# 666DZY666/micronet

Hardware: NVIDIA H100
Metric: qat_step_images_per_sec (higher is better)
Workload: dtype f32 (bf16 tensor-core products of exact integer levels / exact bf16 pieces, fp32 accumulate)

## Files before the change

### include/micronet_b200.h

```cpp
#ifndef MICRONET_B200_H
#define MICRONET_B200_H

#include <stdint.h>

#ifdef __cplusplus
extern "C" {
#endif

typedef void* mnb_stream_t;

#define MNB_E_ARG (-1)
#define MNB_E_UNSUPPORTED (-2)

int mnb_version(void);
const char* mnb_last_error(void);
int64_t mnb_launch_count(void);

typedef struct {
  int32_t batch, in_c, in_h, in_w;
  int32_t out_c, ker_h, ker_w;
  int32_t stride_h, stride_w, pad_h, pad_w, dil_h, dil_w, groups;
} mnb_conv_shape;

#define MNB_ACT_DOREFA 1
// ... 218 lines not shown
                           const mnb_act_qparams* qp, int32_t relu, float* out, const mnb_pk_post* post, mnb_stream_t stream);
int mnb_pk_conv_post_plan(const mnb_conv_shape* s, int32_t terms_a, int32_t terms_w, int32_t cpu, const mnb_pk_post* post,
                          int32_t* out, int32_t n);
int64_t mnb_pk_i8_act_bytes(int32_t batch, int32_t channels, int32_t h, int32_t w);
int mnb_pk_i8_pack_act(const float* x, int32_t batch, int32_t channels, int32_t h, int32_t w, const mnb_act_qparams* qp,
                       int32_t phase_split, int32_t relu, void* out_pk, mnb_stream_t stream);
int mnb_pk_i8_conv_plan(const mnb_conv_shape* s, int32_t* out, int32_t n);
int64_t mnb_pk_i8_wimage_bytes(const mnb_conv_shape* s);
int mnb_pk_i8_pack_weight(const mnb_conv_shape* s, const int16_t* w_int, void* w_img, mnb_stream_t stream);
int mnb_pk_i8_conv(const mnb_conv_shape* s, const void* a_pk, const void* w_img, const float* n_scale, const float* a_scale,
                   float a_scale_const, const float* bias, float* out, const mnb_pk_post* post, int32_t* err_flag,
                   mnb_stream_t stream);
int mnb_quant_add_pack_i8_fwd(const float* a, const float* b, int32_t batch, int32_t channels, int32_t h, int32_t w,
                              const mnb_act_qparams* qp, int32_t relu, float* out, const mnb_pk_post* post, mnb_stream_t stream);
int mnb_bn_relu_quant_pack_i8_fwd(const float* x, int32_t batch, int32_t channels, int32_t hw, const float* mean,
                                  const float* invstd, const float* gamma, const float* beta, const mnb_act_qparams* qp,
                                  int32_t out_shuffle_groups, void* x_packed, mnb_stream_t stream);
int mnb_pk_plane_maxpool(const void* in_pk, int32_t batch, int32_t channels, int32_t h, int32_t w, int32_t k, int32_t s, int32_t p,
                         int32_t int8, void* out_pk, mnb_stream_t stream);
int mnb_pk_plane_maxpool_requant(const void* in_pk, int32_t batch, int32_t channels, int32_t h, int32_t w, int32_t k, int32_t s,
                                 int32_t p, int32_t int8, const mnb_act_qparams* q_in, const mnb_act_qparams* q_out, void* out_pk,
                                 mnb_stream_t stream);
int mnb_pk_plane_maxpool_terms(const void* in_pk, int32_t batch, int32_t channels, int32_t h, int32_t w, int32_t k, int32_t s,
                               int32_t p, int32_t terms, void* out_pk, mnb_stream_t stream);
int mnb_bn_relu_pack_terms_fwd(const float* x, int32_t batch, int32_t channels, int32_t hw, const float* mean,
                               const float* invstd, const float* gamma, const float* beta, int32_t relu,
                               int32_t out_shuffle_groups, int32_t terms, void* x_packed, mnb_stream_t stream);
int64_t mnb_pk_wgrad_scratch_bytes(const mnb_conv_shape* s, int32_t terms_dy, int32_t terms_x);
int mnb_pk_wgrad(const mnb_conv_shape* s, const void* dy_pk, int32_t terms_dy, const void* x_pk, int32_t terms_x,
                 const float* a_scale, const float* kdiv, float* dw, void* scratch, int32_t* err_flag, mnb_stream_t stream);
int mnb_pk_wgrad_taps_plan(const mnb_conv_shape* s, int32_t terms_dy, int32_t terms_x, int32_t* out, int32_t n);
int mnb_pk_wgrad_taps(const mnb_conv_shape* s, const void* dy_pk, int32_t terms_dy, const void* x_pk, int32_t terms_x,
                      const float* a_scale, const float* kdiv, float* dw, void* scratch, int32_t* err_flag, mnb_stream_t stream);
int mnb_pk_gc3_plan(const mnb_conv_shape* s, int32_t mode, int32_t terms_a, int32_t terms_w, int32_t* out, int32_t n);
int mnb_pk_gc3_conv(const mnb_conv_shape* s, int32_t mode, const void* a_pk, int32_t terms_a, const void* w_img, int32_t terms_w,
                    const float* n_scale, const float* a_scale, float a_scale_const, const float* bias, const uint8_t* bits8,
                    float gain, float* out, int32_t* err_flag, mnb_stream_t stream);
int mnb_pk_gc3_conv_codes(const mnb_conv_shape* s, const void* a_pk, int32_t terms_a, const void* w_img, int32_t terms_w,
                          const float* n_scale, const float* a_scale, float a_scale_const, const float* bias, int32_t level_bound,
                          int16_t* codes, float* dec, int32_t* err_flag, mnb_stream_t stream);

int mnb_xnor_supported(const mnb_conv_shape* s);
int64_t mnb_xnor_act_bytes(int32_t batch, int32_t channels, int32_t h, int32_t w, int32_t groups);
int mnb_xnor_pack_act(const float* x, int32_t batch, int32_t channels, int32_t h, int32_t w, int32_t groups, void* out_bits,
                      mnb_stream_t stream);
int64_t mnb_xnor_wimage_bytes(const mnb_conv_shape* s);
int mnb_xnor_pack_weight(const mnb_conv_shape* s, const int16_t* w_int, void* w_img, mnb_stream_t stream);
int mnb_xnor_conv_fwd(const mnb_conv_shape* s, const void* a_bits, const void* w_img, const float* alpha, const float* bias,
                      float* y, mnb_stream_t stream);
#define MNB_XNOR_BITS 0
#define MNB_XNOR_PM1_BF16 1
typedef struct mnb_xnor_post {
  int32_t format;
  int32_t out_groups;
  int32_t shuffle_groups;
  int32_t pool2;
  const float* bn_mean;
  const float* bn_invstd;
  const float* bn_gamma;
  const float* bn_beta;
} mnb_xnor_post;
int64_t mnb_xnor_post_bytes(const mnb_conv_shape* s, const mnb_xnor_post* post);
int mnb_xnor_conv_post(const mnb_conv_shape* s, const void* a_bits, const void* w_img, const float* alpha, const float* bias,
                       const mnb_xnor_post* post, void* out, mnb_stream_t stream);
int mnb_xnor_pack_act_post(const float* x, int32_t batch, int32_t channels, int32_t h, int32_t w, const mnb_xnor_post* post,
                           void* out_bits, mnb_stream_t stream);
// ... 38 lines not shown
```

### micronet_b200/_lib.py

```python
from __future__ import annotations

import ctypes as C
import os

import torch

_HERE = os.path.dirname(os.path.abspath(__file__))
LIB_PATH = os.path.join(_HERE, "lib", "libmicronet_b200.so")

ACT_DOREFA, ACT_IAO, ACT_SIGN = 1, 2, 3


class ConvShape(C.Structure):
    _fields_ = [(n, C.c_int32) for n in (
        "batch", "in_c", "in_h", "in_w", "out_c", "ker_h", "ker_w", "stride_h", "stride_w",
        "pad_h", "pad_w", "dil_h", "dil_w", "groups")]


class ActQParams(C.Structure):
    _fields_ = [("mode", C.c_int32), ("bits", C.c_int32), ("qmin", C.c_int32), ("qmax", C.c_int32),
                ("q_type", C.c_int32), ("scale", C.c_void_p), ("zero_point", C.c_void_p),
                ("obs_min", C.c_void_p), ("obs_max", C.c_void_p)]


# ... 83 lines not shown
    "mnb_pk_pack_weight": (C.c_int, [_SHAPE, _I, _I, _I, _P, _P, _P, _P, _P]),
    "mnb_pk_conv": (C.c_int, [_SHAPE, _I, _P, _I, _P, _I, _P, _P, C.c_float, _P, _P, C.c_float, _P, _P, _P]),
    "mnb_bn_sign_bwd_pack": (C.c_int, [_P, _P, _P, _I, _I, _I, _P, _P, _P, _P, _P, _I, _P, _I, _P, _P, _P]),
    "mnb_bn_sign_pool_bwd_pack": (C.c_int, [_P, _P, _P, _P, _I, _I, _I, _I, _P, _P, _P, _P, _P, _I, _P, _I, _P, _P]),
    "mnb_pk_conv_post": (C.c_int, [_SHAPE, _P, _I, _P, _I, _P, _P, C.c_float, _P, _P, C.POINTER(PkPost), _P, _P]),
    "mnb_pk_conv_post_plan": (C.c_int, [_SHAPE, _I, _I, _I, C.POINTER(PkPost), _P, _I]),
    "mnb_pk_conv_codes": (C.c_int, [_SHAPE, _P, _I, _P, _I, _P, _P, C.c_float, _P, _I, _P, _P, _P, _P]),
    "mnb_codes_decode": (C.c_int, [_P, _P, _I, _I, _I, _P, _P]),
    "mnb_bn_batch_stats_codes": (C.c_int, [_P, _P, _I, _I, _I, _D, _D, _P, _P, _P, _P, _P, _P]),
    "mnb_bn_sign_fwd_packed_codes": (C.c_int, [_P, _P, _I, _I, _I, _P, _P, _P, _P, _I, _P, _P, _P, _P]),
    "mnb_bn_sign_bwd_codes": (C.c_int, [_P, _P, _P, _P, _I, _I, _I, _P, _P, _P, _I, _I, _P, _P, _P, _P, _P, _P]),
    "mnb_bn_sign_pool_fwd_codes": (C.c_int, [_P, _P, _I, _I, _I, _I, _P, _P, _P, _P, _I, _P, _P, _P, _P]),
    "mnb_bn_sign_pool_bwd_codes": (C.c_int, [_P, _P, _P, _P, _P, _I, _I, _I, _I, _P, _P, _P, _I, _I, _P, _P, _P, _P, _P, _P]),
    "mnb_bn_sign_bwd_pack_codes": (C.c_int, [_P, _P, _P, _P, _I, _I, _I, _P, _P, _P, _P, _P, _I, _P, _I, _P, _P, _P]),
    "mnb_bn_sign_pool_bwd_pack_codes": (C.c_int, [_P, _P, _P, _P, _P, _I, _I, _I, _I, _P, _P, _P, _P, _P, _I, _P, _I, _P,
                                                  _P]),
    "mnb_quant_add_pack_fwd": (C.c_int, [_P, _P, _I, _I, _I, _I, _ACTQ, _I, _P, C.POINTER(PkPost), _P]),
    "mnb_pk_i8_act_bytes": (_L, [_I, _I, _I, _I]),
    "mnb_pk_i8_pack_act": (C.c_int, [_P, _I, _I, _I, _I, _ACTQ, _I, _I, _P, _P]),
    "mnb_pk_i8_conv_plan": (C.c_int, [_SHAPE, _P, _I]),
    "mnb_pk_i8_wimage_bytes": (_L, [_SHAPE]),
    "mnb_pk_i8_pack_weight": (C.c_int, [_SHAPE, _P, _P, _P]),
    "mnb_pk_i8_conv": (C.c_int, [_SHAPE, _P, _P, _P, _P, C.c_float, _P, _P, C.POINTER(PkPost), _P, _P]),
    "mnb_quant_add_pack_i8_fwd": (C.c_int, [_P, _P, _I, _I, _I, _I, _ACTQ, _I, _P, C.POINTER(PkPost), _P]),
    "mnb_bn_relu_quant_pack_i8_fwd": (C.c_int, [_P, _I, _I, _I, _P, _P, _P, _P, _ACTQ, _I, _P, _P]),
    "mnb_pk_plane_maxpool": (C.c_int, [_P, _I, _I, _I, _I, _I, _I, _I, _I, _P, _P]),
    "mnb_pk_plane_maxpool_requant": (C.c_int, [_P, _I, _I, _I, _I, _I, _I, _I, _I, _ACTQ, _ACTQ, _P, _P]),
    "mnb_pk_plane_maxpool_terms": (C.c_int, [_P, _I, _I, _I, _I, _I, _I, _I, _I, _P, _P]),
    "mnb_bn_relu_pack_terms_fwd": (C.c_int, [_P, _I, _I, _I, _P, _P, _P, _P, _I, _I, _I, _P, _P]),
    "mnb_pk_wgrad_scratch_bytes": (_L, [_SHAPE, _I, _I]),
    "mnb_pk_wgrad": (C.c_int, [_SHAPE, _P, _I, _P, _I, _P, _P, _P, _P, _P, _P]),
    "mnb_pk_wgrad_taps_plan": (C.c_int, [_SHAPE, _I, _I, _P, _I]),
    "mnb_pk_wgrad_taps": (C.c_int, [_SHAPE, _P, _I, _P, _I, _P, _P, _P, _P, _P, _P]),
    "mnb_pk_gc3_plan": (C.c_int, [_SHAPE, _I, _I, _I, _P, _I]),
    "mnb_pk_gc3_conv": (C.c_int, [_SHAPE, _I, _P, _I, _P, _I, _P, _P, C.c_float, _P, _P, C.c_float, _P, _P, _P]),
    "mnb_pk_gc3_conv_codes": (C.c_int, [_SHAPE, _P, _I, _P, _I, _P, _P, C.c_float, _P, _I, _P, _P, _P, _P]),
    "mnb_xnor_supported": (C.c_int, [_SHAPE]),
    "mnb_xnor_act_bytes": (_L, [_I, _I, _I, _I, _I]),
    "mnb_xnor_pack_act": (C.c_int, [_P, _I, _I, _I, _I, _I, _P, _P]),
    "mnb_xnor_wimage_bytes": (_L, [_SHAPE]),
    "mnb_xnor_pack_weight": (C.c_int, [_SHAPE, _P, _P, _P]),
    "mnb_xnor_conv_fwd": (C.c_int, [_SHAPE, _P, _P, _P, _P, _P, _P]),
    "mnb_xnor_post_bytes": (_L, [_SHAPE, C.POINTER(XnorPost)]),
    "mnb_xnor_conv_post": (C.c_int, [_SHAPE, _P, _P, _P, _P, C.POINTER(XnorPost), _P, _P]),
    "mnb_xnor_pack_act_post": (C.c_int, [_P, _I, _I, _I, _I, C.POINTER(XnorPost), _P, _P]),
    "mnb_xnor_plan": (C.c_int, [_SHAPE, C.POINTER(XnorPost), _P]),
    "mnb_b1_supported": (C.c_int, [_SHAPE]),
    "mnb_b1_act_bytes": (_L, [_I, _I, _I, _I, _I]),
    "mnb_b1_pack_act": (C.c_int, [_P, _I, _I, _I, _I, _I, _P, _P]),
    "mnb_b1_pack_act_post": (C.c_int, [_P, _I, _I, _I, _I, C.POINTER(XnorPost), _P, _P]),
    "mnb_b1_wimage_bytes": (_L, [_SHAPE]),
    "mnb_b1_pack_weight": (C.c_int, [_SHAPE, _P, _P, _P]),
    "mnb_b1_conv_fwd": (C.c_int, [_SHAPE, _P, _P, _P, _P, _P, _P, _P]),
    "mnb_b1_plan": (C.c_int, [_SHAPE, C.POINTER(XnorPost), _P]),
    "mnb_b1_post_bytes": (_L, [_SHAPE, C.POINTER(XnorPost)]),
    "mnb_b1_conv_post": (C.c_int, [_SHAPE, _P, _P, _P, _P, C.POINTER(XnorPost), _P, _P, _P]),
    "mnb_b1_plane_maxpool": (C.c_int, [_P, _I, _I, _I, _I, _I, _I, _I, _I, _P, _P]),
    "mnb_set_tc_profile_buffer": (None, [_P]),
    "mnb_selftest_mma_rate": (C.c_int, [_I, _I, _I, _I, _I, _P, _P, _P]),
    "mnb_selftest_umma": (C.c_int, [_P, _P, _P, _I, _I, _I, _P, _P]),
    "mnb_selftest_tma3d": (C.c_int, [_P, C.POINTER(C.c_int64), C.POINTER(C.c_int32), C.POINTER(C.c_int32), _P, _P, _P]),
}

_lib = None


# ... 42 lines not shown
            raise TypeError(f"micronet_b200: fp32 tensors only (the reference's QAT modules are fp32), got {t.dtype}")


def launch_count() -> int:
    return int(load().mnb_launch_count())


_errflags = {}


def tc_err_flag(device):
    key = (device.type, device.index)
    if key not in _errflags:
        _errflags[key] = torch.zeros(1, dtype=torch.int32, device=device)
    return _errflags[key]


def tc_check(device=None):
    for key, flag in _errflags.items():
        code = int(flag.item())
        if code:
            raise RuntimeError(f"micronet_b200: tensor-core pipeline wait timed out (code {code}) on {key}")


E_UNSUPPORTED = -2
KEEP_DEBUG = False
USE_TC = os.environ.get("MNB_DISABLE_TC", "0") != "1"
PK_MODE = os.environ.get("MNB_PK", "auto")
PK_TERMS = int(os.environ.get("MNB_PK_TERMS", "3"))
PK_TERMS_BWD = int(os.environ.get("MNB_PK_TERMS_BWD", "2"))
PK_WBWTAB = os.environ.get("MNB_PK_WBWTAB", "1") == "1"
PK_WG_TAPS = os.environ.get("MNB_PK_WG_TAPS", "1") != "0"
PK_GC3 = os.environ.get("MNB_PK_GC3", "1") != "0"

XNOR_MODE = os.environ.get("MNB_XNOR", "auto")

PLANE_ONLY = os.environ.get("MNB_PLANE_ONLY", "1") == "1"

_scratch = {}


def scratch(device, rows=1):
    lib = load()
    need = int(lib.mnb_observe_scratch_bytes(0, int(rows)))
    key = (device.type, device.index)
    buf = _scratch.get(key)
    if buf is None or buf.numel() < need:
        buf = torch.zeros(max(need, 1 << 20), dtype=torch.uint8, device=device)
        _scratch[key] = buf
    return buf
```

### micronet_b200/csrc/mnb_pk.cu

```cuda
#include <cuda.h>
#include <cuda_bf16.h>

#include <algorithm>
#include <cstdlib>
#include <cstring>

#include "mnb_common.cuh"
#include "mnb_tc.cuh"

namespace pk {

constexpr int MAXST = 8;
constexpr int MAXTAP = 64, MAXTMPL = 16, MAXY = 4, MAXPAIR = 6, MAXPROG = 512;
constexpr int kSmemBudget = 227 * 1024 - 3072;
constexpr int kNtSizes[] = {16, 32, 48, 64, 96, 128};

struct Tmpl { int kph, tap0, ntap, blk_off, blk_bytes; };

struct Plan {
  int mode;
  int B, G, R, S, stride;
  int HA, WA, C8A, nkph;
  int kg, ng, NOUT;
  int OHr, OWr, OH, OW, omul, ny;
// ... 1703 lines not shown
      const uint32_t nsubs = min(p.NI, p.nsub - stg * p.NI);
      tc::wg_fence();
#pragma unroll
      for (int t = 0; t < kTapsN; ++t) tc::fence_acc(acc[t]);
      for (uint32_t si = 0; si < nsubs; ++si) {
        const uint32_t s16 = slot * p.stage16 + si * p.sub16;
        for (uint32_t j = 0; j < p.ksteps; ++j) {
          for (uint32_t pr = 0; pr < p.npairs; ++pr) {
            const uint64_t ad = a_hi | (uint64_t)(a_lo0 + s16 + 16u * j + p.pair_a16[pr]);
            const uint32_t bb = b_lo0 + s16 + 16u * j + p.pair_b16[pr];
#pragma unroll
            for (int t = 0; t < kTapsN; ++t) tc::Mma<32>::bf16<1, 1>(acc[t], ad, b_hi | (uint64_t)(bb + p.tap16[t]), 1);
          }
        }
      }
      tc::wg_commit();
      tc::wg_wait<0>();
#pragma unroll
      for (int t = 0; t < kTapsN; ++t) tc::fence_acc(acc[t]);
      __syncwarp();
      if (lane == 0) tc::mbar_arrive(&sh.empty[slot]);
      if (++slot == p.nstage) { slot = 0; ph ^= 1u; }
    }
    float* dst = p.partial + ((int64_t)split * gridDim.x + blk) * (int64_t)(kTapsN * 64 * 128);
    const int kr = 64 * wg + 16 * w4 + (lane >> 2), cb = 32 * wg + 2 * (lane & 3);
#pragma unroll
    for (int t = 0; t < kTapsN; ++t)
#pragma unroll
      for (int j = 0; j < 4; ++j) {
        if ((j >> 1) != (w4 >> 1)) continue;
#pragma unroll
        for (int e = 0; e < 4; ++e) dst[(int64_t)(t * 64 + cb + 8 * j + (e & 1)) * 128 + kr + 8 * (e >> 1)] = acc[t][4 * j + e];
      }
  }
  __syncthreads();
}

constexpr int kGc3MaxMb = 8;
constexpr int kGc3MaxProg = 128;
constexpr int kGc3Cons = 3;
constexpr int kGc3Threads = 128 * (1 + kGc3Cons);
constexpr int kGc3SmemBudget = 227 * 1024 - 4096;
constexpr int kGc3TmaRegs = 40, kGc3MmaRegs = 152;
__host__ __device__ constexpr int gc3_max_mb(int nt) { return nt == 32 ? 6 : kGc3MaxMb; }

struct Gc3Plan {
  Plan pl;
  int GB, nblk, TB, n_tiles, cpb, BW, THH, npos, nmb, plane, SP;
  int a_box_bytes, a_piece_bytes, stage_bytes, nstage, w_bytes, stg_bytes, off_stage, off_stg, off_rowmap, smem_bytes;
  int nprog;
  uint32_t prog[kGc3MaxProg];
  int16_t chain[kGc3MaxProg][4];
};

struct Gc3Params {
  uint32_t prog[kGc3MaxProg];
  int nprog, mode, TA, GB, ng, kg8, NOUT, B, TB, n_tiles, cpb, nmb, npos, BW, THH, OH, OW, plane, SP, C8O, wlo, hlo;
  int a_box_bytes, a_piece_bytes, stage_bytes, nstage, w_bytes, img_bytes, stg_bytes, off_stage, off_stg, off_rowmap, smem_bytes;
  const uint8_t* w_img;
  const float* n_scale;
  const float* a_scale;
  float a_scale_const;
  const float* bias;
  const uint8_t* bits8;
  float gain;
  float* out;
// ... 1022 lines not shown
  if (int e = make_wgt_plan(s, terms_dy, terms_x, pl)) return e;
  WgtParams p;
  memset(&p, 0, sizeof(p));
  p.stg_per_split = pl.stg_per_split; p.nstg_total = pl.nstg_total; p.NI = pl.NI; p.nsub = pl.nsub; p.ksteps = pl.rows_dy / 16;
  p.npairs = pl.npairs; p.nstage = pl.nstage; p.stage16 = pl.stage_bytes >> 4; p.sub16 = pl.sub_bytes >> 4;
  p.dy_sbo = (uint32_t)pl.rows_dy * 16u; p.x_sbo = (uint32_t)pl.rows_x * 16u; p.x_off16 = (pl.TA * pl.dy_bytes) >> 4;
  for (int i = 0; i < pl.npairs; ++i) {
    p.pair_a16[i] = (uint32_t)(pl.pair_a[i] * pl.dy_bytes) >> 4;
    p.pair_b16[i] = (uint32_t)(pl.pair_b[i] * pl.x_bytes) >> 4;
  }
  for (int t = 0; t < kTapsN; ++t) p.tap16[t] = (uint32_t)pl.tap_off[t];
  p.row_tiles = pl.row_tiles; p.TA = pl.TA; p.TX = pl.TX; p.TH = pl.TH; p.hlo = pl.hlo; p.wlo = pl.wlo;
  p.stage_bytes = pl.stage_bytes; p.sub_bytes = pl.sub_bytes; p.dy_bytes = pl.dy_bytes; p.x_bytes = pl.x_bytes;
  p.dy_box_bytes = pl.dy_box_bytes; p.x_box_bytes = pl.x_box_bytes; p.smem_bytes = pl.smem_bytes;
  p.partial = reinterpret_cast<float*>(scratch); p.err = err_flag;
  CUtensorMap tdy[3], tx[3];
  const int64_t dy_plane = (int64_t)pl.B * pl.K8 * pl.P * pl.Q * 16;
  const int64_t x_plane = (int64_t)pl.B * pl.C8X * pl.HX * pl.WX * 16;
  for (int t = 0; t < 3; ++t) {
    if (int e = make_pk_tmap(&tdy[t], dy_pk, dy_plane, t < pl.TA ? t : 0, pl.B, pl.K8, pl.P, pl.Q, pl.BW, pl.TH, 1, 16)) return e;
    if (int e = make_pk_tmap(&tx[t], x_pk, x_plane, t < pl.TX ? t : 0, pl.B, pl.C8X, pl.HX, pl.WX, pl.BW, pl.THH, 1, 8)) return e;
  }
  if (int e = set_max_smem(pk_wgrad_taps_kernel, kSmemBudget)) return e;
  cudaStream_t st = (cudaStream_t)stream;
  pk_wgrad_taps_kernel<<<dim3(pl.G, pl.splits), kWgtThreads, pl.smem_bytes, st>>>(tdy[0], tdy[1], tdy[2], tx[0], tx[1], tx[2], p);
  const dim3 rgrid(kTapsCin * kTapsN, 1, pl.G * kTapsGm);
  wg_reduce_kernel<<<rgrid, 128, 0, st>>>(p.partial, pl.splits, pl.G, kTapsGm, 1, 1, kTapsN, pl.Nc, kTapsCout, kTapsCin, kTapsCout,
                                          kTapsCin, a_scale, kdiv, dw);
  MNB_LAUNCHED(2);
  return 0;
}


extern "C" int mnb_pk_gc3_plan(const mnb_conv_shape* s, int32_t mode, int32_t terms_a, int32_t terms_w, int32_t* out, int32_t n) {
  static pk::Gc3Plan g;
  if (int e = pk::make_gc3_plan(s, mode, terms_a, terms_w, g)) return e;
  if (out) {
    const int v[10] = {g.GB, g.TB, g.nmb, g.nstage, g.smem_bytes, g.nblk * g.cpb, g.n_tiles, g.nprog, g.pl.Nt, pk::kGc3Cons};
    for (int i = 0; i < std::min(n, 10); ++i) out[i] = v[i];
    for (int i = 10; i < n && (i - 10) / 4 < g.nprog; ++i) out[i] = g.chain[(i - 10) / 4][(i - 10) % 4];
  }
  return 0;
}

static int pk_gc3_impl(const mnb_conv_shape* s, int32_t mode, const void* a_pk, int32_t terms_a, const void* w_img, int32_t terms_w,
                       const float* n_scale, const float* a_scale, float a_scale_const, const float* bias, const uint8_t* bits8,
                       float gain, float* out, int16_t* codes, float* dec, int32_t* err_flag, mnb_stream_t stream) {
  using namespace pk;
  MNB_REQUIRE(s && a_pk && w_img && (out != nullptr) != (codes != nullptr) && err_flag, "NULL pk_gc3 pointer");
  static Gc3Plan g;
  if (int e = make_gc3_plan(s, mode, terms_a, terms_w, g)) return e;
  MNB_REQUIRE(g.nstage % kGc3Cons == 0, "pk gc3: %d stages are not a whole number per MMA warpgroup", g.nstage);
  const Plan& pl = g.pl;
  auto al16 = [](const void* q) { return (reinterpret_cast<uintptr_t>(q) & 15) == 0; };
  if (!al16(a_pk) || !al16(w_img) || !al16(out ? (const void*)out : (const void*)codes))
    return mnb_fail(MNB_E_UNSUPPORTED, "pk gc3: operands and output must be 16-byte aligned");
  static Gc3Params p;
  memset(&p, 0, sizeof(p));
  for (int i = 0; i < g.nprog; ++i) p.prog[i] = g.prog[i];
  p.nprog = g.nprog; p.mode = mode; p.TA = terms_a; p.GB = g.GB; p.ng = pl.ng; p.kg8 = pl.kg / 8; p.NOUT = pl.NOUT; p.B = pl.B;
  p.TB = g.TB; p.n_tiles = g.n_tiles; p.cpb = g.cpb; p.nmb = g.nmb; p.npos = g.npos; p.BW = g.BW; p.THH = g.THH; p.OH = pl.OHr;
  p.OW = pl.OWr; p.plane = g.plane; p.SP = g.SP; p.C8O = ceil_div(pl.NOUT, 8); p.wlo = pl.wlo; p.hlo = pl.hlo;
  p.a_box_bytes = g.a_box_bytes; p.a_piece_bytes = g.a_piece_bytes; p.stage_bytes = g.stage_bytes; p.nstage = g.nstage;
  p.w_bytes = g.w_bytes; p.img_bytes = pl.img_bytes[0]; p.stg_bytes = g.stg_bytes; p.off_stage = g.off_stage; p.off_stg = g.off_stg;
  p.off_rowmap = g.off_rowmap; p.smem_bytes = g.smem_bytes;
  p.w_img = reinterpret_cast<const uint8_t*>(w_img);
// ... 38 lines not shown
```

### micronet_b200/functional.py

```python
from __future__ import annotations

import ctypes as C

import torch
from torch.autograd import Function

from . import _lib as L


class KernelTimer:

    def __init__(self):
        self.records = []

    def run(self, kind, sh, fn):
        a, b = torch.cuda.Event(enable_timing=True), torch.cuda.Event(enable_timing=True)
        a.record()
        rc = fn()
        b.record()
        self.records.append((kind, tuple(getattr(sh, f) for f, _ in sh._fields_), a, b))
        return rc

    def summary(self):
        out = {}
# ... 293 lines not shown
            y._mnb_codes = (codes, dec)
    if rc == L.E_UNSUPPORTED:
        rc = _timed("fwd_pk", sh, lambda: PK.run_conv(sh, 0, x_pk, ta, w_img, tw, y,
                                                      n_scale=w_scale if w_int is not None else None, a_scale=a_scale,
                                                      a_scale_const=a_const, bias=bias))
    if rc == L.E_UNSUPPORTED:
        return False
    L.check(rc, "pk_conv fwd")
    ctx.pk_x, ctx.pk_ta, ctx.pk_bits8, ctx.pk_prepacked = x_pk, ta, bits8, prepacked is not None
    ctx.pk_gain = 0.1 if (spec is not None and spec.mode == L.ACT_DOREFA) else 1.0
    ctx.pk_wg_scale = None
    if spec is not None:
        ctx.pk_wg_scale = a_scale if spec.mode == L.ACT_IAO else _dorefa_scale_tensor(spec.bits, x.device)
    if spec is None and w_int is not None and need_dw and not PK.padded(sh.out_c, sh.groups):
        y._mnb_pk_conv = (w_scale if need_dx else None, Tb)
    return True


def _pk_backward(ctx, dy):
    from . import pk as PK
    sh = ctx.sh
    T = min(L.PK_TERMS, L.PK_TERMS_BWD)
    int_w = ctx.w_int is not None
    need_dx, need_dw = ctx.needs_input_grad[0], ctx.needs_input_grad[1]
    fold = int_w and need_dx
    pre = getattr(dy, "_mnb_pk_dy", None)
    if pre is not None:
        if pre[1] != T or (pre[2] is not None) != fold or PK.padded(sh.out_c, sh.groups):
            raise RuntimeError("micronet_b200: packed gradient operand does not match this layer's backward configuration")
        dy_pk = pre[0]
    else:
        dy_pk, _ = PK.pack_act(dy, None, T, ch_scale=ctx.w_scale if fold else None, groups=sh.groups)
    dx = dwq = None
    if need_dx:
        tw = 1 if int_w else T
        w_img = PK.pack_weight(sh, 1, T, tw, w_int=ctx.w_int, w_f32=None if int_w else ctx.wq,
                               kzero=ctx.w_scale if int_w else None)
        dx = torch.empty((sh.batch, sh.in_c, sh.in_h, sh.in_w), dtype=torch.float32, device=dy.device)
        plain_gain = ctx.pk_gain if ctx.pk_prepacked else 1.0
        L.check(_timed("dgrad_pk", sh, lambda: PK.run_conv(sh, 1, dy_pk, T, w_img, tw, dx, bits8=ctx.pk_bits8, gain=ctx.pk_gain,
                                                           a_scale_const=plain_gain)), "pk_conv dgrad")
    if need_dw:
        dwq = torch.empty_like(ctx.wq)
        tx = min(ctx.pk_ta, T)
        kdiv = ctx.w_scale if fold else None
        L.check(_timed("wgrad_pk", sh, lambda: PK.run_wgrad(sh, dy_pk, T, ctx.pk_x, tx, dwq, a_scale=ctx.pk_wg_scale,
                                                            kdiv=kdiv)), "pk_wgrad")
    return dx, dwq


def _xnor_forward(x, w_int, w_scale, bias, sh, y, groups):
    from . import xnor as XN
    if not (XN.supported(sh) and (L.XNOR_MODE == "all" or xnor_preferred(sh, getattr(x, "_mnb_pk_pm1", None) is not None))):
        return False
    a_bits = XN.pack_act(materialized(x), groups)
    rc = _timed("fwd_xnor", sh, lambda: XN.conv(sh, a_bits, XN.pack_weight(sh, w_int), y, alpha=w_scale, bias=bias))
    if rc == L.E_UNSUPPORTED:
        return False
    L.check(rc, "xnor_conv_fwd")
    return True


def _save_unpacked(ctx, x, spec, codes, bits, keep_x):
    if spec is not None and (ctx.needs_input_grad[0] or ctx.needs_input_grad[1]):
        spec = spec.frozen()
    ctx.spec, ctx.codes, ctx.bits = spec, codes, bits
    ctx.x = x if keep_x else None


def _act_operands(spec, codes, x):
    ops = L.ConvOperands()
    if codes is None:
        ops.a_f32 = x.data_ptr()
        return ops
    ops.a_codes, ops.a_offset = codes.data_ptr(), spec.code_offset
    if spec.mode == L.ACT_IAO:
        ops.a_offset_zp, ops.a_scale = L.ptr(spec.zero_point), L.ptr(spec.scale)
    elif spec.mode == L.ACT_DOREFA:
# ... 559 lines not shown
```

### micronet_b200/pk.py

```python
from __future__ import annotations

import ctypes as C

import torch

from . import _lib as L

_plan_cache = {}


def _key(sh):
    return tuple(getattr(sh, f) for f, _ in sh._fields_)


def supported(sh, mode, terms_a, terms_w):
    k = ("c", _key(sh), mode, terms_a, terms_w)
    if k not in _plan_cache:
        _plan_cache[k] = L.load().mnb_pk_conv_plan(C.byref(sh), mode, terms_a, terms_w, None) == 0
    return _plan_cache[k]


def segmented(sh, mode, terms_a, terms_w):
    k = ("s", _key(sh), mode, terms_a, terms_w)
    if k not in _plan_cache:
# ... 211 lines not shown
    lib = L.load()
    nbytes = int(lib.mnb_pk_wgrad_scratch_bytes(C.byref(sh), terms_dy, terms_x))
    if nbytes < 0:
        return L.E_UNSUPPORTED
    ws = torch.empty(max(nbytes, 16), dtype=torch.uint8, device=dw.device)
    return lib.mnb_pk_wgrad(C.byref(sh), dy_pk.data_ptr(), terms_dy, x_pk.data_ptr(), terms_x, L.ptr(a_scale),
                            L.ptr(kdiv), dw.data_ptr(), ws.data_ptr(), L.tc_err_flag(dw.device).data_ptr(), L.stream())


def wgrad_taps_plan(sh, terms_dy, terms_x):
    k = ("wt", _key(sh), terms_dy, terms_x)
    if k not in _plan_cache:
        out = (C.c_int32 * 12)()
        ok = L.load().mnb_pk_wgrad_taps_plan(C.byref(sh), terms_dy, terms_x, out, 12) == 0
        names = ("blocks", "splits", "NI", "nstage", "BW", "TH", "stg_per_split", "smem_bytes", "acc_regs")
        plan = None
        if ok:
            plan = dict(zip(names, out[:9]))
            plan["scratch_bytes"] = out[9] | (out[10] << 31)
            plan["npairs"] = out[11]
        _plan_cache[k] = plan
    return _plan_cache[k]


def wgrad_taps(sh, dy_pk, terms_dy, x_pk, terms_x, dw, a_scale=None, kdiv=None):
    plan = wgrad_taps_plan(sh, terms_dy, terms_x)
    if plan is None:
        return L.E_UNSUPPORTED
    ws = torch.empty(plan["scratch_bytes"], dtype=torch.uint8, device=dw.device)
    return L.load().mnb_pk_wgrad_taps(C.byref(sh), dy_pk.data_ptr(), terms_dy, x_pk.data_ptr(), terms_x, L.ptr(a_scale),
                                      L.ptr(kdiv), dw.data_ptr(), ws.data_ptr(), L.tc_err_flag(dw.device).data_ptr(), L.stream())


def gc3_plan(sh, mode, terms_a, terms_w):
    k = ("g3", _key(sh), mode, terms_a, terms_w)
    if k not in _plan_cache:
        out = (C.c_int32 * (10 + 4 * 128))()
        ok = L.load().mnb_pk_gc3_plan(C.byref(sh), mode, terms_a, terms_w, out, len(out)) == 0
        plan = None
        if ok:
            names = ("groups_per_block", "images_per_tile", "m_blocks", "nstage", "smem_bytes", "ctas", "tiles", "chain_len",
                     "Nt", "mma_warpgroups")
            plan = dict(zip(names, out[:10]))
            plan["chain"] = [tuple(out[10 + 4 * i:14 + 4 * i]) for i in range(plan["chain_len"])]
        _plan_cache[k] = plan
    return _plan_cache[k]


def gc3_conv(sh, mode, a_pk, terms_a, w_img, terms_w, out, n_scale=None, a_scale=None, a_scale_const=1.0, bias=None,
             bits8=None, gain=1.0):
    return L.load().mnb_pk_gc3_conv(C.byref(sh), mode, a_pk.data_ptr(), terms_a, w_img.data_ptr(), terms_w, L.ptr(n_scale),
                                    L.ptr(a_scale), float(a_scale_const), L.ptr(bias), L.ptr(bits8), float(gain),
                                    out.data_ptr(), L.tc_err_flag(out.device).data_ptr(), L.stream())


def gc3_conv_codes(sh, a_pk, w_img, codes, dec, n_scale=None, a_scale=None, a_scale_const=1.0, bias=None, level_bound=1):
    return L.load().mnb_pk_gc3_conv_codes(C.byref(sh), a_pk.data_ptr(), 1, w_img.data_ptr(), 1, L.ptr(n_scale), L.ptr(a_scale),
                                          float(a_scale_const), L.ptr(bias), int(level_bound), codes.data_ptr(), dec.data_ptr(),
                                          L.tc_err_flag(codes.device).data_ptr(), L.stream())


def run_conv(sh, mode, a_pk, terms_a, w_img, terms_w, out, **epilogue):
    if L.PK_GC3 and gc3_plan(sh, mode, terms_a, terms_w) is not None:
        rc = gc3_conv(sh, mode, a_pk, terms_a, w_img, terms_w, out, **epilogue)
        if rc != L.E_UNSUPPORTED:
            return rc
    return conv(sh, mode, a_pk, terms_a, w_img, terms_w, out, **epilogue)


def run_conv_codes(sh, a_pk, w_img, codes, dec, **epilogue):
    if L.PK_GC3 and gc3_plan(sh, 0, 1, 1) is not None:
        rc = gc3_conv_codes(sh, a_pk, w_img, codes, dec, **epilogue)
        if rc != L.E_UNSUPPORTED:
            return rc
    return conv_codes(sh, a_pk, w_img, codes, dec, **epilogue)


def run_wgrad(sh, dy_pk, terms_dy, x_pk, terms_x, dw, a_scale=None, kdiv=None):
    fn = wgrad_taps if L.PK_WG_TAPS and wgrad_taps_plan(sh, terms_dy, terms_x) is not None else wgrad
    return fn(sh, dy_pk, terms_dy, x_pk, terms_x, dw, a_scale=a_scale, kdiv=kdiv)
```

Measured before the change: 41270.

## Fuse 1x1 conv data-gradient and weight-gradient into one warp-specialized kernel

```diff
diff --git a/harness/pk_bwd1x1_probe.py b/harness/pk_bwd1x1_probe.py
--- /dev/null
+++ b/harness/pk_bwd1x1_probe.py
@@ -0,0 +1,74 @@
+import argparse
+import json
+
+import torch
+
+from harness.wgrad_taps_probe import card
+from micronet_b200 import _lib as L, pk as PK
+
+SHAPES = {"L1/L2 256->256 g2 @32": (256, 256, 32, 32, 256, 2), "L4/L5 512->512 g4 @16": (256, 512, 16, 16, 512, 4),
+          "L7 1024->1024 g8 @8": (256, 1024, 8, 8, 1024, 8)}
+
+
+def main():
+    ap = argparse.ArgumentParser()
+    ap.add_argument("--iters", type=int, default=50)
+    ap.add_argument("--rounds", type=int, default=5)
+    args = ap.parse_args()
+    dev = torch.device("cuda:0")
+    out = {"card": card(), "layers": {}}
+    for name, (B, Cc, H, W, K, G) in SHAPES.items():
+        sh = L.ConvShape(B, Cc, H, W, K, 1, 1, 1, 1, 0, 0, 1, 1, G)
+        plan = PK.bwd1x1_plan(sh, 2, 1, 1)
+        g = torch.Generator().manual_seed(7)
+        ops = []
+        for _ in range(4):
+            dy = torch.randn(B, K, H, W, generator=g).to(dev)
+            x = torch.randint(0, 2, (B, Cc, H, W), generator=g).float().mul_(2).sub_(1).to(dev)
+            w_int = torch.randint(-1, 2, (K, Cc // G, 1, 1), generator=g).to(torch.int16).to(dev)
+            ops.append((PK.pack_act(dy, None, 2, groups=G)[0], PK.pack_act(x, None, 1, groups=G)[0],
+                        PK.pack_weight(sh, 1, 2, 1, w_int=w_int)))
+        res = {k: (torch.empty(B, Cc, H, W, device=dev), torch.empty(K, Cc // G, 1, 1, device=dev)) for k in ("sep", "fused")}
+
+        def sep(dy_pk, x_pk, w_img, dx, dw):
+            L.check(PK.conv(sh, 1, dy_pk, 2, w_img, 1, dx, a_scale_const=0.25), "pk_conv dgrad")
+            L.check(PK.wgrad(sh, dy_pk, 2, x_pk, 1, dw), "pk_wgrad")
+
+        def fused(dy_pk, x_pk, w_img, dx, dw):
+            L.check(PK.bwd1x1(sh, dy_pk, 2, x_pk, 1, w_img, 1, dx, dw, a_scale_const=0.25), "pk_bwd1x1")
+
+        fns = {"sep": sep, "fused": fused}
+
+        def window(k):
+            a, b = torch.cuda.Event(enable_timing=True), torch.cuda.Event(enable_timing=True)
+            a.record()
+            for i in range(args.iters):
+                fns[k](*ops[i % 4], *res[k])
+            b.record()
+            torch.cuda.synchronize()
+            return a.elapsed_time(b) * 1e3 / args.iters
+
+        for k in fns:
+            window(k)
+        t = {k: [] for k in fns}
+        for _ in range(args.rounds):
+            for k in fns:
+                t[k].append(window(k))
+        L.tc_check()
+        med = {k: sorted(v)[len(v) // 2] for k, v in t.items()}
+        n_out = B * K * H * W
+        dy_b, x_b, dx_b = n_out * 4, B * Cc * H * W * 2, B * Cc * H * W * 4
+        w_b = ops[0][2].numel()
+        part_b = plan["scratch_bytes"] * 2
+        bytes_ = {"sep": 2 * dy_b + x_b + w_b + dx_b + part_b, "fused": dy_b + x_b + w_b + dx_b + part_b}
+        same = all(torch.equal(res["sep"][i].view(torch.int32), res["fused"][i].view(torch.int32)) for i in range(2))
+        out["layers"][name] = {
+            "sep_us": med["sep"], "fused_us": med["fused"], "speedup": med["sep"] / med["fused"],
+            "sep_GBps": bytes_["sep"] / med["sep"] * 1e-3, "fused_GBps": bytes_["fused"] / med["fused"] * 1e-3,
+            "sep_bytes": bytes_["sep"], "fused_bytes": bytes_["fused"],
+            "sep_windows_us": t["sep"], "fused_windows_us": t["fused"], "byte_equal": same, "plan": plan}
+    print(json.dumps(out, indent=1))
+
+
+if __name__ == "__main__":
+    main()
diff --git a/include/micronet_b200.h b/include/micronet_b200.h
--- a/include/micronet_b200.h
+++ b/include/micronet_b200.h
@@ -274,6 +274,10 @@
 int mnb_pk_wgrad_taps_plan(const mnb_conv_shape* s, int32_t terms_dy, int32_t terms_x, int32_t* out, int32_t n);
 int mnb_pk_wgrad_taps(const mnb_conv_shape* s, const void* dy_pk, int32_t terms_dy, const void* x_pk, int32_t terms_x,
                       const float* a_scale, const float* kdiv, float* dw, void* scratch, int32_t* err_flag, mnb_stream_t stream);
+int mnb_pk_bwd1x1_plan(const mnb_conv_shape* s, int32_t terms_dy, int32_t terms_x, int32_t terms_w, int32_t* out, int32_t n);
+int mnb_pk_bwd1x1(const mnb_conv_shape* s, const void* dy_pk, int32_t terms_dy, const void* x_pk, int32_t terms_x,
+                  const void* w_img, int32_t terms_w, float a_scale_const, const uint8_t* bits8, float gain, float* dx,
+                  const float* a_scale, const float* kdiv, float* dw, void* scratch, int32_t* err_flag, mnb_stream_t stream);
 int mnb_pk_gc3_plan(const mnb_conv_shape* s, int32_t mode, int32_t terms_a, int32_t terms_w, int32_t* out, int32_t n);
 int mnb_pk_gc3_conv(const mnb_conv_shape* s, int32_t mode, const void* a_pk, int32_t terms_a, const void* w_img, int32_t terms_w,
                     const float* n_scale, const float* a_scale, float a_scale_const, const float* bias, const uint8_t* bits8,
diff --git a/micronet_b200/_lib.py b/micronet_b200/_lib.py
--- a/micronet_b200/_lib.py
+++ b/micronet_b200/_lib.py
@@ -139,6 +139,8 @@
     "mnb_pk_wgrad": (C.c_int, [_SHAPE, _P, _I, _P, _I, _P, _P, _P, _P, _P, _P]),
     "mnb_pk_wgrad_taps_plan": (C.c_int, [_SHAPE, _I, _I, _P, _I]),
     "mnb_pk_wgrad_taps": (C.c_int, [_SHAPE, _P, _I, _P, _I, _P, _P, _P, _P, _P, _P]),
+    "mnb_pk_bwd1x1_plan": (C.c_int, [_SHAPE, _I, _I, _I, _P, _I]),
+    "mnb_pk_bwd1x1": (C.c_int, [_SHAPE, _P, _I, _P, _I, _P, _I, C.c_float, _P, C.c_float, _P, _P, _P, _P, _P, _P, _P]),
     "mnb_pk_gc3_plan": (C.c_int, [_SHAPE, _I, _I, _I, _P, _I]),
     "mnb_pk_gc3_conv": (C.c_int, [_SHAPE, _I, _P, _I, _P, _I, _P, _P, C.c_float, _P, _P, C.c_float, _P, _P, _P]),
     "mnb_pk_gc3_conv_codes": (C.c_int, [_SHAPE, _P, _I, _P, _I, _P, _P, C.c_float, _P, _I, _P, _P, _P, _P]),
@@ -247,6 +249,7 @@
 PK_WBWTAB = os.environ.get("MNB_PK_WBWTAB", "1") == "1"
 PK_WG_TAPS = os.environ.get("MNB_PK_WG_TAPS", "1") != "0"
 PK_GC3 = os.environ.get("MNB_PK_GC3", "1") != "0"
+PK_BWD1X1 = os.environ.get("MNB_PK_BWD1X1", "1") != "0"
 
 XNOR_MODE = os.environ.get("MNB_XNOR", "auto")
 
diff --git a/micronet_b200/csrc/mnb_pk.cu b/micronet_b200/csrc/mnb_pk.cu
--- a/micronet_b200/csrc/mnb_pk.cu
+++ b/micronet_b200/csrc/mnb_pk.cu
@@ -1759,6 +1759,192 @@
 #pragma unroll
         for (int e = 0; e < 4; ++e) dst[(int64_t)(t * 64 + cb + 8 * j + (e & 1)) * 128 + kr + 8 * (e >> 1)] = acc[t][4 * j + e];
       }
+  }
+  __syncthreads();
+}
+
+constexpr int kBwdThreads = 384;
+constexpr int kBwdRows = 64;
+constexpr int kBwdProg = 64;
+constexpr int kBwdTmaRegs = 40, kBwdMmaRegs = 232;
+
+struct BwdPlan {
+  WgPlan wg;
+  Plan dg;
+  int nprog, off_w, w_bytes, nstage, smem_bytes;
+};
+
+static int make_bwd_plan(const mnb_conv_shape* s, int TA, int TX, int TW, BwdPlan& b) {
+  MNB_REQUIRE(s != nullptr, "conv shape is NULL");
+  MNB_REQUIRE(TA >= 1 && TA <= 3 && TX >= 1 && TX <= 3 && TW >= 1 && TW <= 3, "term counts must be 1..3");
+  memset(&b, 0, sizeof(b));
+  const int C = s->in_c, K = s->out_c, G = s->groups;
+  MNB_REQUIRE(s->batch > 0 && C > 0 && K > 0 && s->in_h > 0 && s->in_w > 0 && G > 0 && C % G == 0 && K % G == 0,
+              "bad conv shape");
+  auto no = [](const char* why) { return mnb_fail(MNB_E_UNSUPPORTED, "pk bwd1x1: %s", why); };
+  if (s->ker_h != 1 || s->ker_w != 1) return no("filter is not 1x1");
+  if (s->stride_h != 1 || s->stride_w != 1 || s->dil_h != 1 || s->dil_w != 1) return no("stride or dilation != 1");
+  if (s->pad_h != 0 || s->pad_w != 0) return no("padding != 0");
+  if (C / G > 128 || K / G > 128) return no("more than 128 channels per group");
+  if (G > 1 && ((C / G) % 8 || (K / G) % 8)) return no("group-padded operand planes");
+  if (int e = make_wg_plan(s, TA, TX, b.wg)) return e;
+  if (int e = make_plan(s, 1, TA, TW, b.dg)) return e;
+  const WgPlan& w = b.wg;
+  const Plan& d = b.dg;
+  if (w.gm != 1 || w.n_ktiles != 1 || w.n_ctiles != 1 || w.n_tg != 1) return no("weight-gradient block is not one whole group");
+  if (w.rows_dy != kBwdRows) return no("sub-block raster is not 64 positions");
+  if (d.n_ntiles != 1 || d.Nt != w.Nc || d.Nt % 32) return no("data-gradient N tile differs from the weight-gradient tile");
+  if (d.segmented) return no("segmented data-gradient plan");
+  if (d.chunks * d.ksteps * 16 > 128) return no("data-gradient K-steps beyond the dy box");
+  b.nprog = d.chunks * d.npairs * d.ksteps;
+  if (d.ny != 1 || d.ntmpl[0] != 1 || b.nprog > kBwdProg)
+    return mnb_fail(MNB_E_ARG, "pk bwd1x1: data-gradient plan with %d templates, %d MMAs", d.ntmpl[0], b.nprog);
+  b.w_bytes = round_up(d.img_bytes[0], 1024);
+  b.nstage = std::min(MAXST, (kSmemBudget - 1024 - b.w_bytes) / w.stage_bytes);
+  if (b.nstage < 2) return no("fewer than two stages fit next to the weight image");
+  b.off_w = b.nstage * w.stage_bytes + 1024;
+  b.smem_bytes = b.off_w + b.w_bytes;
+  return 0;
+}
+
+struct BwdParams {
+  uint32_t stg_per_split, nstg_total, NI, nsub, ksteps, npairs, nstage, stage16, sub16, dy_sbo, x_sbo, x_off16;
+  uint32_t pair_a16[MAXPAIR], pair_b16[MAXPAIR];
+  int row_tiles, TA, TX, TH, stage_bytes, sub_bytes, dy_bytes, x_bytes, dy_box_bytes, x_box_bytes, smem_bytes, cout_g8, cin_g8;
+  float* partial;
+  uint32_t nprog, dg_lbo, w_lbo, off_w, w_bytes, img_bytes;
+  uint32_t prog[kBwdProg];
+  const uint8_t* w_img;
+  int B, P, Q, BW, C, cin_g, C8O;
+  float a_scale_const, gain;
+  float bias0;
+  const uint8_t* bits8;
+  float* dx;
+  int* err;
+};
+
+template <int NC>
+__global__ void __launch_bounds__(kBwdThreads, 1)
+pk_bwd1x1_kernel(const __grid_constant__ CUtensorMap dy0, const __grid_constant__ CUtensorMap dy1,
+                 const __grid_constant__ CUtensorMap dy2, const __grid_constant__ CUtensorMap x0,
+                 const __grid_constant__ CUtensorMap x1, const __grid_constant__ CUtensorMap x2,
+                 const __grid_constant__ BwdParams p) {
+  extern __shared__ __align__(1024) uint8_t smem[];
+  __shared__ WgShared sh;
+  __shared__ uint64_t wbar;
+  const int tid = threadIdx.x, warp = tid >> 5, lane = tid & 31;
+  if (tid == 0) {
+    for (int i = 0; i < MAXST; ++i) { tc::mbar_init(&sh.full[i], 1); tc::mbar_init(&sh.empty[i], 8); }
+    tc::mbar_init(&wbar, 1);
+    sh.abort = 0;
+    tc::fence_barrier_init();
+    tc::prefetch_tmap(&dy0); tc::prefetch_tmap(&x0);
+  }
+  for (int i = tid; i < (int)p.off_w / 16; i += kBwdThreads) reinterpret_cast<uint4*>(smem)[i] = make_uint4(0, 0, 0, 0);
+  tc::fence_proxy_async_smem();
+  __syncthreads();
+  const int g = blockIdx.x, split = blockIdx.y;
+  const uint32_t stg0 = (uint32_t)split * p.stg_per_split, stg1 = min(p.nstg_total, stg0 + p.stg_per_split);
+
+  if (warp < 4) {
+    asm volatile("setmaxnreg.dec.sync.aligned.u32 %0;" ::"n"(kBwdTmaRegs));
+    if (warp == 0 && lane == 0) {
+      tc::mbar_arrive_expect_tx(&wbar, p.img_bytes);
+      tc::bulk_load_1d(smem + p.off_w, p.w_img + (size_t)g * p.img_bytes, p.img_bytes, &wbar);
+      uint32_t slot = 0, ph = 0;
+      const int k8 = g * p.cout_g8, c8 = g * p.cin_g8;
+      for (uint32_t stg = stg0; stg < stg1; ++stg) {
+        if (!tc::mbar_wait(&sh.empty[slot], ph ^ 1u, p.err, 731)) break;
+        const int sub0 = (int)(stg * p.NI), nsubs = min((int)p.NI, (int)p.nsub - sub0);
+        tc::mbar_arrive_expect_tx(&sh.full[slot], (uint32_t)(nsubs * (p.TA * p.dy_box_bytes + p.TX * p.x_box_bytes)));
+        for (int si = 0; si < nsubs; ++si) {
+          const int sub = sub0 + si;
+          const int b = sub / p.row_tiles, h0 = (sub - b * p.row_tiles) * p.TH;
+          uint8_t* sb = smem + (size_t)slot * p.stage_bytes + (size_t)si * p.sub_bytes;
+          tc::tma_load_4d(sb, &dy0, &sh.full[slot], 0, h0, b, k8);
+          if (p.TA > 1) tc::tma_load_4d(sb + p.dy_bytes, &dy1, &sh.full[slot], 0, h0, b, k8);
+          if (p.TA > 2) tc::tma_load_4d(sb + 2 * p.dy_bytes, &dy2, &sh.full[slot], 0, h0, b, k8);
+          uint8_t* xb = sb + (size_t)p.TA * p.dy_bytes;
+          tc::tma_load_4d(xb, &x0, &sh.full[slot], 0, h0, b, c8);
+          if (p.TX > 1) tc::tma_load_4d(xb + p.x_bytes, &x1, &sh.full[slot], 0, h0, b, c8);
+          if (p.TX > 2) tc::tma_load_4d(xb + 2 * p.x_bytes, &x2, &sh.full[slot], 0, h0, b, c8);
+        }
+        if (++slot == p.nstage) { slot = 0; ph ^= 1u; }
+      }
+    }
+  } else {
+    asm volatile("setmaxnreg.inc.sync.aligned.u32 %0;" ::"n"(kBwdMmaRegs));
+    constexpr int NR = NC / 2, ND = NC / 2, NRD = ND / 2;
+    const int wg = (warp - 4) >> 2, w4 = (warp - 4) & 3;
+    const uint64_t a_desc0 = tc::smem_desc_mnmajor_noswz(tc::smem_u32(smem), 128, p.dy_sbo) + (uint64_t)((8u * wg * p.dy_sbo) >> 4);
+    const uint64_t b_desc0 = tc::smem_desc_mnmajor_noswz(tc::smem_u32(smem), 128, p.x_sbo) + (uint64_t)p.x_off16;
+    const uint64_t da_desc0 = tc::smem_desc_kmajor_noswz(tc::smem_u32(smem), p.dg_lbo, 128);
+    const uint64_t db_desc0 = tc::smem_desc_kmajor_noswz(tc::smem_u32(smem + p.off_w), p.w_lbo, 128) + (uint64_t)(ND * wg);
+    const uint32_t a_lo0 = (uint32_t)a_desc0, b_lo0 = (uint32_t)b_desc0, da_lo0 = (uint32_t)da_desc0, db_lo0 = (uint32_t)db_desc0;
+    const uint64_t a_hi = a_desc0 & 0xffffffff00000000ull, b_hi = b_desc0 & 0xffffffff00000000ull;
+    const uint64_t da_hi = da_desc0 & 0xffffffff00000000ull, db_hi = db_desc0 & 0xffffffff00000000ull;
+    const int64_t plane = (int64_t)p.P * p.Q;
+    const int n_lo = ND * wg + 2 * (lane & 3);
+    float acc[NR], dacc[NRD];
+    tc::zero_acc(acc);
+    tc::mbar_wait_soft(&wbar, 0, p.err, 733, &sh.abort);
+    uint32_t slot = 0, ph = 0;
+    for (uint32_t stg = stg0; stg < stg1; ++stg) {
+      tc::mbar_wait_soft(&sh.full[slot], ph, p.err, 732, &sh.abort);
+      const uint32_t nsubs = min(p.NI, p.nsub - stg * p.NI);
+      for (uint32_t si = 0; si < nsubs; ++si) {
+        const uint32_t s16 = slot * p.stage16 + si * p.sub16;
+        tc::zero_acc(dacc);
+        tc::wg_fence();
+        tc::fence_acc(acc);
+        tc::fence_acc(dacc);
+        for (uint32_t j = 0; j < p.ksteps; ++j)
+          for (uint32_t pr = 0; pr < p.npairs; ++pr)
+            tc::Mma<NC>::template bf16<1, 1>(acc, a_hi | (uint64_t)(a_lo0 + s16 + 16u * j + p.pair_a16[pr]),
+                                             b_hi | (uint64_t)(b_lo0 + s16 + 16u * j + p.pair_b16[pr]), 1);
+        for (uint32_t e = 0; e < p.nprog; ++e) {
+          const uint32_t w = p.prog[e];
+          tc::Mma<ND>::template bf16<0, 0>(dacc, da_hi | (uint64_t)(da_lo0 + s16 + (w & 0xffffu)),
+                                           db_hi | (uint64_t)(db_lo0 + (w >> 16)), 1);
+        }
+        tc::wg_commit();
+        tc::wg_wait<0>();
+        tc::fence_acc(acc);
+        tc::fence_acc(dacc);
+        const int sub = (int)((stg * p.NI) + si);
+        const int b = sub / p.row_tiles, h0 = (sub - b * p.row_tiles) * p.TH;
+#pragma unroll
+        for (int i = 0; i < 2; ++i) {
+          const int m = 16 * w4 + (lane >> 2) + 8 * i;
+          const int oh = h0 + m / p.BW, ow = m - (m / p.BW) * p.BW;
+          if (oh >= p.P || ow >= p.Q) continue;
+          float* orow = p.dx + ((int64_t)b * p.C + g * p.cin_g) * plane + (int64_t)oh * p.Q + ow;
+          const uint8_t* brow = p.bits8 ? p.bits8 + ((int64_t)b * p.C8O + g * (p.cin_g >> 3)) * plane + (int64_t)oh * p.Q + ow : nullptr;
+#pragma unroll
+          for (int j = 0; j < ND / 8; ++j) {
+            const int n = n_lo + 8 * j;
+            if (n >= p.cin_g) continue;
+            if (brow) {
+              const uint32_t mk = __ldg(brow + (int64_t)(n >> 3) * plane) >> (n & 7);
+              orow[(int64_t)n * plane] = (mk & 1u) ? dacc[4 * j + 2 * i] * p.gain : 0.f;
+              if (n + 1 < p.cin_g) orow[(int64_t)(n + 1) * plane] = (mk & 2u) ? dacc[4 * j + 2 * i + 1] * p.gain : 0.f;
+            } else {
+              orow[(int64_t)n * plane] = fmaf(dacc[4 * j + 2 * i], p.a_scale_const, p.bias0);
+              if (n + 1 < p.cin_g) orow[(int64_t)(n + 1) * plane] = fmaf(dacc[4 * j + 2 * i + 1], p.a_scale_const, p.bias0);
+            }
+          }
+        }
+      }
+      __syncwarp();
+      if (lane == 0) tc::mbar_arrive(&sh.empty[slot]);
+      if (++slot == p.nstage) { slot = 0; ph ^= 1u; }
+    }
+    float* dst = p.partial + ((int64_t)split * gridDim.x + g) * (int64_t)(NC * 128);
+    const int fr = 64 * wg + 16 * w4 + (lane >> 2), fc = 2 * (lane & 3);
+#pragma unroll
+    for (int j = 0; j < NR / 4; ++j)
+#pragma unroll
+      for (int e = 0; e < 4; ++e) dst[(int64_t)(8 * j + fc + (e & 1)) * 128 + fr + 8 * (e >> 1)] = acc[4 * j + e];
   }
   __syncthreads();
 }
@@ -2847,6 +3033,85 @@
 }
 
 
+extern "C" int mnb_pk_bwd1x1_plan(const mnb_conv_shape* s, int32_t terms_dy, int32_t terms_x, int32_t terms_w, int32_t* out,
+                                  int32_t n) {
+  pk::BwdPlan b;
+  if (int e = pk::make_bwd_plan(s, terms_dy, terms_x, terms_w, b)) return e;
+  if (out) {
+    const pk::WgPlan& w = b.wg;
+    const int64_t sb = w.partial_floats * 4;
+    const int v[15] = {w.G, w.splits, w.NI, b.nstage, w.BW, w.TH, w.stg_per_split, b.smem_bytes, w.nsub, w.nstg_total, b.nprog,
+                       (int)(sb & 0x7fffffff), (int)(sb >> 31), w.npairs, w.Nc};
+    for (int i = 0; i < std::min(n, 15); ++i) out[i] = v[i];
+  }
+  return 0;
+}
+
+extern "C" int mnb_pk_bwd1x1(const mnb_conv_shape* s, const void* dy_pk, int32_t terms_dy, const void* x_pk, int32_t terms_x,
+                             const void* w_img, int32_t terms_w, float a_scale_const, const uint8_t* bits8, float gain, float* dx,
+                             const float* a_scale, const float* kdiv, float* dw, void* scratch, int32_t* err_flag,
+                             mnb_stream_t stream) {
+  using namespace pk;
+  MNB_REQUIRE(s && dy_pk && x_pk && w_img && dx && dw && scratch && err_flag, "NULL pk_bwd1x1 pointer");
+  BwdPlan b;
+  if (int e = make_bwd_plan(s, terms_dy, terms_x, terms_w, b)) return e;
+  const WgPlan& pl = b.wg;
+  const Plan& d = b.dg;
+  static BwdParams p;
+  memset(&p, 0, sizeof(p));
+  p.stg_per_split = pl.stg_per_split; p.nstg_total = pl.nstg_total; p.NI = pl.NI; p.nsub = pl.nsub; p.ksteps = pl.rows_dy / 16;
+  p.npairs = pl.npairs; p.nstage = b.nstage; p.stage16 = pl.stage_bytes >> 4; p.sub16 = pl.sub_bytes >> 4;
+  p.dy_sbo = (uint32_t)pl.rows_dy * 16u; p.x_sbo = (uint32_t)pl.rows_x * 16u; p.x_off16 = (pl.TA * pl.dy_bytes) >> 4;
+  for (int i = 0; i < pl.npairs; ++i) {
+    p.pair_a16[i] = (uint32_t)(pl.pair_a[i] * pl.dy_bytes) >> 4;
+    p.pair_b16[i] = (uint32_t)(pl.pair_b[i] * pl.x_bytes) >> 4;
+  }
+  p.row_tiles = pl.row_tiles; p.TA = pl.TA; p.TX = pl.TX; p.TH = pl.TH;
+  p.stage_bytes = pl.stage_bytes; p.sub_bytes = pl.sub_bytes; p.dy_bytes = pl.dy_bytes; p.x_bytes = pl.x_bytes;
+  p.dy_box_bytes = pl.dy_box_bytes; p.x_box_bytes = pl.x_box_bytes; p.smem_bytes = b.smem_bytes;
+  p.cout_g8 = pl.cout_g / 8; p.cin_g8 = pl.cin_g / 8;
+  p.partial = reinterpret_cast<float*>(scratch);
+  p.nprog = (uint32_t)b.nprog;
+  {
+    const int b_tap16 = (d.CC / 8) * d.Nt, blk16 = d.tmpl[0][0].blk_bytes >> 4;
+    int e = 0;
+    for (int cc = 0; cc < d.chunks; ++cc)
+      for (int pr = 0; pr < d.npairs; ++pr)
+        for (int j = 0; j < d.ksteps; ++j) {
+          const uint32_t a16 = (uint32_t)(d.pair_a[pr] * pl.dy_bytes / 16 + (cc * d.ksteps + j) * 2 * pl.rows_dy);
+          const uint32_t b16 = (uint32_t)(cc * blk16 + d.pair_b[pr] * b_tap16 + j * 2 * d.Nt);
+          if (a16 > 0xffffu || b16 > 0xffffu) return mnb_fail(MNB_E_ARG, "pk bwd1x1: MMA program offset overflow");
+          p.prog[e++] = a16 | (b16 << 16);
+        }
+  }
+  p.dg_lbo = (uint32_t)pl.rows_dy * 16u; p.w_lbo = (uint32_t)d.Nt * 16u; p.off_w = (uint32_t)b.off_w;
+  p.w_bytes = (uint32_t)b.w_bytes; p.img_bytes = (uint32_t)d.img_bytes[0];
+  p.w_img = reinterpret_cast<const uint8_t*>(w_img);
+  p.B = pl.B; p.P = pl.P; p.Q = pl.Q; p.BW = pl.BW; p.C = s->in_c; p.cin_g = s->in_c / s->groups;
+  p.C8O = s->groups * ceil_div(p.cin_g, 8);
+  p.a_scale_const = a_scale_const; p.gain = gain; p.bias0 = 0.f; p.bits8 = bits8; p.dx = dx; p.err = err_flag;
+  CUtensorMap tdy[3], tx[3];
+  const int64_t dy_plane = (int64_t)pl.B * pl.K8 * pl.P * pl.Q * 16;
+  const int64_t x_plane = (int64_t)pl.B * pl.C8X * pl.HX * pl.WX * 16;
+  for (int t = 0; t < 3; ++t) {
+    if (int e = make_pk_tmap(&tdy[t], dy_pk, dy_plane, t < pl.TA ? t : 0, pl.B, pl.K8, pl.P, pl.Q, pl.BW, pl.TH, 1, 16)) return e;
+    if (int e = make_pk_tmap(&tx[t], x_pk, x_plane, t < pl.TX ? t : 0, pl.B, pl.C8X, pl.HX, pl.WX, pl.BW, pl.THH, 1, pl.Nc / 8)) return e;
+  }
+  using BwdFn = void (*)(const CUtensorMap, const CUtensorMap, const CUtensorMap, const CUtensorMap, const CUtensorMap,
+                         const CUtensorMap, const BwdParams);
+  static const BwdFn fns[4] = {pk_bwd1x1_kernel<32>, pk_bwd1x1_kernel<64>, pk_bwd1x1_kernel<96>, pk_bwd1x1_kernel<128>};
+  const BwdFn fn = fns[pl.Nc / 32 - 1];
+  if (int e = set_max_smem(fn, kSmemBudget)) return e;
+  cudaStream_t st = (cudaStream_t)stream;
+  fn<<<dim3(pl.G, pl.splits), kBwdThreads, b.smem_bytes, st>>>(tdy[0], tdy[1], tdy[2], tx[0], tx[1], tx[2], p);
+  const dim3 rgrid(pl.cin_o, 1, pl.G);
+  wg_reduce_kernel<<<rgrid, 128, 0, st>>>(p.partial, pl.splits, pl.G, 1, 1, 1, 1, pl.Nc, pl.cout_o, pl.cin_o, pl.cout_g, pl.cin_g,
+                                          a_scale, kdiv, dw);
+  MNB_LAUNCHED(2);
+  return 0;
+}
+
+
 extern "C" int mnb_pk_gc3_plan(const mnb_conv_shape* s, int32_t mode, int32_t terms_a, int32_t terms_w, int32_t* out, int32_t n) {
   static pk::Gc3Plan g;
   if (int e = pk::make_gc3_plan(s, mode, terms_a, terms_w, g)) return e;
diff --git a/micronet_b200/functional.py b/micronet_b200/functional.py
--- a/micronet_b200/functional.py
+++ b/micronet_b200/functional.py
@@ -349,18 +349,25 @@
     else:
         dy_pk, _ = PK.pack_act(dy, None, T, ch_scale=ctx.w_scale if fold else None, groups=sh.groups)
     dx = dwq = None
+    tw = 1 if int_w else T
+    tx = min(ctx.pk_ta, T)
+    kdiv = ctx.w_scale if fold else None
+    plain_gain = ctx.pk_gain if ctx.pk_prepacked else 1.0
     if need_dx:
-        tw = 1 if int_w else T
         w_img = PK.pack_weight(sh, 1, T, tw, w_int=ctx.w_int, w_f32=None if int_w else ctx.wq,
                                kzero=ctx.w_scale if int_w else None)
         dx = torch.empty((sh.batch, sh.in_c, sh.in_h, sh.in_w), dtype=torch.float32, device=dy.device)
-        plain_gain = ctx.pk_gain if ctx.pk_prepacked else 1.0
+    if need_dx and need_dw and pre is not None and PK.bwd1x1_taken(sh, T, tx, tw):
+        dwq = torch.empty_like(ctx.wq)
+        L.check(_timed("bwd1x1_pk", sh, lambda: PK.run_bwd(sh, dy_pk, T, ctx.pk_x, tx, w_img, tw, dx, dwq, bits8=ctx.pk_bits8,
+                                                           gain=ctx.pk_gain, a_scale_const=plain_gain,
+                                                           a_scale=ctx.pk_wg_scale, kdiv=kdiv)), "pk_bwd1x1")
+        return dx, dwq
+    if need_dx:
         L.check(_timed("dgrad_pk", sh, lambda: PK.run_conv(sh, 1, dy_pk, T, w_img, tw, dx, bits8=ctx.pk_bits8, gain=ctx.pk_gain,
                                                            a_scale_const=plain_gain)), "pk_conv dgrad")
     if need_dw:
         dwq = torch.empty_like(ctx.wq)
-        tx = min(ctx.pk_ta, T)
-        kdiv = ctx.w_scale if fold else None
         L.check(_timed("wgrad_pk", sh, lambda: PK.run_wgrad(sh, dy_pk, T, ctx.pk_x, tx, dwq, a_scale=ctx.pk_wg_scale,
                                                             kdiv=kdiv)), "pk_wgrad")
     return dx, dwq
diff --git a/micronet_b200/pk.py b/micronet_b200/pk.py
--- a/micronet_b200/pk.py
+++ b/micronet_b200/pk.py
@@ -267,6 +267,33 @@
                                       L.ptr(kdiv), dw.data_ptr(), ws.data_ptr(), L.tc_err_flag(dw.device).data_ptr(), L.stream())
 
 
+def bwd1x1_plan(sh, terms_dy, terms_x, terms_w):
+    k = ("b1", _key(sh), terms_dy, terms_x, terms_w)
+    if k not in _plan_cache:
+        out = (C.c_int32 * 15)()
+        ok = L.load().mnb_pk_bwd1x1_plan(C.byref(sh), terms_dy, terms_x, terms_w, out, 15) == 0
+        plan = None
+        if ok:
+            names = ("groups", "splits", "NI", "nstage", "BW", "TH", "stg_per_split", "smem_bytes", "nsub", "nstg_total",
+                     "dgrad_chain")
+            plan = dict(zip(names, out[:11]))
+            plan["scratch_bytes"] = out[11] | (out[12] << 31)
+            plan["npairs"], plan["Nc"] = out[13], out[14]
+        _plan_cache[k] = plan
+    return _plan_cache[k]
+
+
+def bwd1x1(sh, dy_pk, terms_dy, x_pk, terms_x, w_img, terms_w, dx, dw, bits8=None, gain=1.0, a_scale_const=1.0, a_scale=None,
+           kdiv=None):
+    plan = bwd1x1_plan(sh, terms_dy, terms_x, terms_w)
+    if plan is None:
+        return L.E_UNSUPPORTED
+    ws = torch.empty(plan["scratch_bytes"], dtype=torch.uint8, device=dw.device)
+    return L.load().mnb_pk_bwd1x1(C.byref(sh), dy_pk.data_ptr(), terms_dy, x_pk.data_ptr(), terms_x, w_img.data_ptr(), terms_w,
+                                  float(a_scale_const), L.ptr(bits8), float(gain), dx.data_ptr(), L.ptr(a_scale), L.ptr(kdiv),
+                                  dw.data_ptr(), ws.data_ptr(), L.tc_err_flag(dw.device).data_ptr(), L.stream())
+
+
 def gc3_plan(sh, mode, terms_a, terms_w):
     k = ("g3", _key(sh), mode, terms_a, terms_w)
     if k not in _plan_cache:
@@ -314,3 +341,18 @@
 def run_wgrad(sh, dy_pk, terms_dy, x_pk, terms_x, dw, a_scale=None, kdiv=None):
     fn = wgrad_taps if L.PK_WG_TAPS and wgrad_taps_plan(sh, terms_dy, terms_x) is not None else wgrad
     return fn(sh, dy_pk, terms_dy, x_pk, terms_x, dw, a_scale=a_scale, kdiv=kdiv)
+
+
+def bwd1x1_taken(sh, terms_dy, terms_x, terms_w):
+    return L.PK_BWD1X1 and bwd1x1_plan(sh, terms_dy, terms_x, terms_w) is not None
+
+
+def run_bwd(sh, dy_pk, terms_dy, x_pk, terms_x, w_img, terms_w, dx, dw, bits8=None, gain=1.0, a_scale_const=1.0, a_scale=None,
+            kdiv=None):
+    if bwd1x1_taken(sh, terms_dy, terms_x, terms_w):
+        return bwd1x1(sh, dy_pk, terms_dy, x_pk, terms_x, w_img, terms_w, dx, dw, bits8=bits8, gain=gain,
+                      a_scale_const=a_scale_const, a_scale=a_scale, kdiv=kdiv)
+    rc = run_conv(sh, 1, dy_pk, terms_dy, w_img, terms_w, dx, bits8=bits8, gain=gain, a_scale_const=a_scale_const)
+    if rc != 0:
+        return rc
+    return run_wgrad(sh, dy_pk, terms_dy, x_pk, terms_x, dw, a_scale=a_scale, kdiv=kdiv)
```

Measured after the change: 43850 (median of 6 runs). +6.3%, better.
